# Kamino666/video_features

Measured on NVIDIA H100. Metric: frames/sec CLIP-ViT-B/32 @224px, higher is better.
Workload: dtype f16

## Files before the change

video_features_b200/csrc/attn_gemm.cu:

```cuda
#include <string.h>

#include <atomic>

#include "common.cuh"
#include "internal.h"
#include "wgmma.cuh"

namespace vf {

namespace {

constexpr int BM = 128, BK = 64, BN = 192, STAGES = 4;
constexpr int FRAMES_PER_TILE = 2, TOK = 50, TILE_ROWS = FRAMES_PER_TILE * TOK;
constexpr int THREADS = 384, CONSUMER_THREADS = 256, CONSUMER_WARPS = 8;
constexpr uint32_t A_BYTES = BM * BK * 2, B_BYTES = BN * BK * 2, STAGE_BYTES = A_BYTES + B_BYTES;
constexpr int PITCH = 200;
constexpr uint32_t STG_BYTES = BM * PITCH * 2;
constexpr uint32_t ZERO_BYTES = 128;
constexpr uint32_t BAR_BYTES = 2 * STAGES * 8;
constexpr uint32_t SMEM_BYTES = STAGES * STAGE_BYTES + STG_BYTES + ZERO_BYTES + BAR_BYTES + 1024;
static_assert(SMEM_BYTES <= 227 * 1024, "shared memory budget");

__device__ __forceinline__ void mma16816(float* c, const uint32_t* a, uint32_t b0, uint32_t b1) {
    asm volatile(
        "mma.sync.aligned.m16n8k16.row.col.f32.f16.f16.f32 {%0,%1,%2,%3}, {%4,%5,%6,%7}, {%8,%9}, {%0,%1,%2,%3};"
        : "+f"(c[0]), "+f"(c[1]), "+f"(c[2]), "+f"(c[3])
        : "r"(a[0]), "r"(a[1]), "r"(a[2]), "r"(a[3]), "r"(b0), "r"(b1));
}
__device__ __forceinline__ void ldsm_x4(uint32_t* r, const void* p) {
    asm volatile("ldmatrix.sync.aligned.m8n8.x4.shared.b16 {%0,%1,%2,%3}, [%4];"
                 : "=r"(r[0]), "=r"(r[1]), "=r"(r[2]), "=r"(r[3]) : "r"(smem_u32(p)));
}
__device__ __forceinline__ void ldsm_x4_trans(uint32_t* r, const void* p) {
    asm volatile("ldmatrix.sync.aligned.m8n8.x4.trans.shared.b16 {%0,%1,%2,%3}, [%4];"
                 : "=r"(r[0]), "=r"(r[1]), "=r"(r[2]), "=r"(r[3]) : "r"(smem_u32(p)));
}
__device__ __forceinline__ void attention_unit(__half* S, const __half* zero, int qrow0, int krow0, int nvalid, int lane) {
    const int g = lane >> 2, t = lane & 3;
    uint32_t aq[4][4];
#pragma unroll
    for (int ks = 0; ks < 4; ++ks) ldsm_x4(aq[ks], S + (qrow0 + (lane & 15)) * PITCH + ks * 16 + (lane >> 4) * 8);
    float s[8][4];
#pragma unroll
    for (int nt = 0; nt < 7; ++nt) {
        s[nt][0] = s[nt][1] = s[nt][2] = s[nt][3] = 0.f;
#pragma unroll
        for (int kp = 0; kp < 2; ++kp) {
            uint32_t bk[4];
            const int kr = nt * 8 + (lane & 7);
            ldsm_x4(bk, kr < TOK ? S + (krow0 + kr) * PITCH + 64 + kp * 32 + (lane >> 3) * 8 : zero);
            mma16816(s[nt], aq[2 * kp], bk[0], bk[1]);
            mma16816(s[nt], aq[2 * kp + 1], bk[2], bk[3]);
        }
    }
    const float sc = 0.125f * 1.4426950408889634f;
    float m_lo = -INFINITY, m_hi = -INFINITY;
#pragma unroll
    for (int nt = 0; nt < 7; ++nt) {
#pragma unroll
        for (int j = 0; j < 2; ++j) {
            const bool valid = nt * 8 + 2 * t + j < TOK;
            s[nt][j] = valid ? s[nt][j] * sc : -INFINITY;
            s[nt][2 + j] = valid ? s[nt][2 + j] * sc : -INFINITY;
            m_lo = fmaxf(m_lo, s[nt][j]);
            m_hi = fmaxf(m_hi, s[nt][2 + j]);
        }
    }
    m_lo = fmaxf(m_lo, __shfl_xor_sync(0xffffffffu, m_lo, 1));
    m_lo = fmaxf(m_lo, __shfl_xor_sync(0xffffffffu, m_lo, 2));
    m_hi = fmaxf(m_hi, __shfl_xor_sync(0xffffffffu, m_hi, 1));
    m_hi = fmaxf(m_hi, __shfl_xor_sync(0xffffffffu, m_hi, 2));
    float sum_lo = 0.f, sum_hi = 0.f;
#pragma unroll
    for (int nt = 0; nt < 7; ++nt) {
#pragma unroll
        for (int j = 0; j < 2; ++j) {
            s[nt][j] = exp2f(s[nt][j] - m_lo);
            s[nt][2 + j] = exp2f(s[nt][2 + j] - m_hi);
            sum_lo += s[nt][j];
            sum_hi += s[nt][2 + j];
        }
    }
    s[7][0] = s[7][1] = s[7][2] = s[7][3] = 0.f;
    sum_lo += __shfl_xor_sync(0xffffffffu, sum_lo, 1);
    sum_lo += __shfl_xor_sync(0xffffffffu, sum_lo, 2);
    sum_hi += __shfl_xor_sync(0xffffffffu, sum_hi, 1);
    sum_hi += __shfl_xor_sync(0xffffffffu, sum_hi, 2);
    const float inv_lo = 1.0f / sum_lo, inv_hi = 1.0f / sum_hi;
    uint32_t pa[4][4];
#pragma unroll
    for (int kk = 0; kk < 4; ++kk) {
        pa[kk][0] = pack_half2(s[2 * kk][0] * inv_lo, s[2 * kk][1] * inv_lo);
        pa[kk][1] = pack_half2(s[2 * kk][2] * inv_hi, s[2 * kk][3] * inv_hi);
        pa[kk][2] = pack_half2(s[2 * kk + 1][0] * inv_lo, s[2 * kk + 1][1] * inv_lo);
        pa[kk][3] = pack_half2(s[2 * kk + 1][2] * inv_hi, s[2 * kk + 1][3] * inv_hi);
    }
    __syncwarp();
#pragma unroll
    for (int np = 0; np < 4; ++np) {
        float o0[4] = {0.f, 0.f, 0.f, 0.f}, o1[4] = {0.f, 0.f, 0.f, 0.f};
#pragma unroll
        for (int kk = 0; kk < 4; ++kk) {
            uint32_t bv[4];
            const int vr = kk * 16 + (lane & 7) + ((lane >> 3) & 1) * 8;
            ldsm_x4_trans(bv, vr < TOK ? S + (krow0 + vr) * PITCH + 128 + np * 16 + (lane >> 4) * 8 : zero);
            mma16816(o0, pa[kk], bv[0], bv[1]);
            mma16816(o1, pa[kk], bv[2], bv[3]);
        }
        if (g < nvalid) {
            *reinterpret_cast<uint32_t*>(S + (qrow0 + g) * PITCH + np * 16 + 2 * t) = pack_half2(o0[0], o0[1]);
            *reinterpret_cast<uint32_t*>(S + (qrow0 + g) * PITCH + np * 16 + 8 + 2 * t) = pack_half2(o1[0], o1[1]);
        }
        if (g + 8 < nvalid) {
            *reinterpret_cast<uint32_t*>(S + (qrow0 + g + 8) * PITCH + np * 16 + 2 * t) = pack_half2(o0[2], o0[3]);
            *reinterpret_cast<uint32_t*>(S + (qrow0 + g + 8) * PITCH + np * 16 + 8 + 2 * t) = pack_half2(o1[2], o1[3]);
        }
    }
    __syncwarp();
}

__global__ void __launch_bounds__(THREADS, 1)
qkv_attention_kernel(const __grid_constant__ CUtensorMap tmA, const __grid_constant__ CUtensorMap tmB,
                     const float* __restrict__ bias, __half* __restrict__ att, const int n_frames, const int heads) {
    extern __shared__ uint8_t smem_raw[];
    uint8_t* smem = reinterpret_cast<uint8_t*>((reinterpret_cast<uintptr_t>(smem_raw) + 1023) & ~uintptr_t(1023));
    uint8_t* sA = smem;
    uint8_t* sB = smem + STAGES * A_BYTES;
    __half* S = reinterpret_cast<__half*>(smem + STAGES * STAGE_BYTES);
    __half* zero = reinterpret_cast<__half*>(smem + STAGES * STAGE_BYTES + STG_BYTES);
    uint64_t* full = reinterpret_cast<uint64_t*>(smem + STAGES * STAGE_BYTES + STG_BYTES + ZERO_BYTES);
    uint64_t* empty = full + STAGES;

    const int warp = threadIdx.x >> 5, lane = threadIdx.x & 31;
    const int num_m = (n_frames + FRAMES_PER_TILE - 1) / FRAMES_PER_TILE;
    const int num_tiles = num_m * heads;
    const int width = heads * 64;
    constexpr int num_k = 768 / BK;

    if (threadIdx.x == 0) {
        tma_prefetch_desc(&tmA);
        tma_prefetch_desc(&tmB);
        for (int i = 0; i < STAGES; ++i) {
            mbar_init(&full[i], 1);
            mbar_init(&empty[i], CONSUMER_WARPS);
        }
        fence_mbar_init();
    }
    if (threadIdx.x < ZERO_BYTES / 16) reinterpret_cast<uint4*>(zero)[threadIdx.x] = make_uint4(0, 0, 0, 0);
    __syncthreads();

    if (warp < 4) {
        if (warp == 0 && lane == 0) {
            int stage = 0;
            uint32_t phase = 0;
            for (int tile = blockIdx.x; tile < num_tiles; tile += gridDim.x) {
                const int m0 = (tile % num_m) * TILE_ROWS;
                const int n0 = (tile / num_m) * BN;
                for (int kk = 0; kk < num_k; ++kk) {
                    mbar_wait(&empty[stage], phase ^ 1);
                    mbar_expect_tx(&full[stage], STAGE_BYTES);
                    tma_load_2d(sA + stage * A_BYTES, &tmA, &full[stage], kk * BK, m0);
                    tma_load_2d(sB + stage * B_BYTES, &tmB, &full[stage], kk * BK, n0);
                    if (++stage == STAGES) { stage = 0; phase ^= 1; }
                }
            }
        }
        return;
    }

    const int wg = (warp >> 2) - 1, wq = warp & 3;
    const int e = warp - 4;
    const int f = e >> 2, tok0 = (e & 3) * 16;
    const int krow0 = TOK * f, qrow0 = krow0 + tok0;
    float acc[BN / 2];
    int stage = 0;
    uint32_t phase = 0;
    for (int tile = blockIdx.x; tile < num_tiles; tile += gridDim.x) {
        const int m_blk = tile % num_m, head = tile / num_m;
        int prev = -1;
        for (int kb = 0; kb < num_k; ++kb) {
            mbar_wait(&full[stage], phase);
            const uint64_t adesc = wgmma_desc_sw128(sA + stage * A_BYTES + wg * (64 * 128));
            const uint64_t bdesc = wgmma_desc_sw128(sB + stage * B_BYTES);
            wgmma_fence_regs<BN / 2>(acc);
            wgmma_fence();
#pragma unroll
            for (int k = 0; k < BK / 16; ++k) Wgmma<BN>::mma(acc, adesc + 2 * k, bdesc + 2 * k, (kb | k) != 0 ? 1u : 0u);
            wgmma_commit();
            wgmma_wait<1>();
            wgmma_fence_regs<BN / 2>(acc);
            if (prev >= 0) {
                __syncwarp();
                if (lane == 0) mbar_arrive(&empty[prev]);
            }
            prev = stage;
            if (++stage == STAGES) { stage = 0; phase ^= 1; }
        }
        wgmma_wait<0>();
        wgmma_fence_regs<BN / 2>(acc);
        __syncwarp();
        if (lane == 0) mbar_arrive(&empty[prev]);

        named_bar_sync(1, CONSUMER_THREADS);
        const float* hb = bias + head * BN;
#pragma unroll
        for (int j = 0; j < BN / 8; ++j) {
            const int c = 8 * j + 2 * (lane & 3);
            const float2 b = __ldg(reinterpret_cast<const float2*>(hb + c));
#pragma unroll
            for (int h = 0; h < 2; ++h) {
                const int r = wg * 64 + wq * 16 + (lane >> 2) + 8 * h;
                *reinterpret_cast<uint32_t*>(S + r * PITCH + c) = pack_half2(acc[4 * j + 2 * h] + b.x, acc[4 * j + 2 * h + 1] + b.y);
            }
        }
        named_bar_sync(1, CONSUMER_THREADS);
        attention_unit(S, zero, qrow0, krow0, tok0 + 16 <= TOK ? 16 : TOK - tok0, lane);
        const int frame = m_blk * FRAMES_PER_TILE + f;
        if (frame < n_frames) {
            __half* orow = att + (int64_t(frame) * TOK) * width + head * 64;
#pragma unroll
            for (int i = 0; i < 4; ++i) {
                const int r = i * 4 + (lane >> 3), seg = lane & 7;
                const int tok = tok0 + r;
                if (tok < TOK)
                    *reinterpret_cast<uint4*>(orow + int64_t(tok) * width + seg * 8) =
                        *reinterpret_cast<const uint4*>(S + (qrow0 + r) * PITCH + seg * 8);
            }
        }
    }
}

}

int qkv_attention(const __half* h, int lda, const __half* w_perm, const float* bias_perm, __half* att, int n_frames, int heads,
                  cudaStream_t stream) {
    if (n_frames <= 0) return VF_OK;
    if (heads * 64 != 768) return fail(VF_ERR_UNSUPPORTED, "qkv_attention: built for width 768 (heads * 64)");
    static std::atomic<bool> attr_set[64];
    int dev = 0;
    VF_CUDA(cudaGetDevice(&dev));
    if (dev < 0 || dev >= 64 || !attr_set[dev].load(std::memory_order_acquire)) {
        VF_CUDA(cudaFuncSetAttribute(qkv_attention_kernel, cudaFuncAttributeMaxDynamicSharedMemorySize, SMEM_BYTES));
        if (dev >= 0 && dev < 64) attr_set[dev].store(true, std::memory_order_release);
    }
    const int M = n_frames * TOK;
    CUtensorMap tmA, tmB;
    VF_TRY(make_tmap_2d(&tmA, h, 2, uint64_t(M), 768, uint64_t(lda) * 2, BM, BK));
    VF_TRY(make_tmap_2d(&tmB, w_perm, 2, uint64_t(heads) * BN, 768, 768 * 2, BN, BK));
    const int tiles = ((n_frames + FRAMES_PER_TILE - 1) / FRAMES_PER_TILE) * heads;
    const int sms = device_sm_count();
    const int grid = tiles < sms ? tiles : sms;
    qkv_attention_kernel<<<grid, THREADS, SMEM_BYTES, stream>>>(tmA, tmB, bias_perm, att, n_frames, heads);
    VF_CUDA(cudaGetLastError());
    return VF_OK;
}

}
```

Before: 46370.

## Warp-specialize fused QKV-attention kernel with MMA/attention overlap via staging ring

Splits the consumer role into one MMA warpgroup, which computes full 128-row QKV tiles with two accumulators, and two attention warpgroups. They hand off through a double-buffered shared-memory ring guarded by staged/freed mbarriers, so the GEMM for the next tile runs while attention works on the previous one. Tiles now pack contiguous frames (128 rows instead of 100), and each CTA is pinned to one head over a contiguous frame range, so the weight slice and bias (now cached in shared memory) stay resident. Register budgets are rebalanced with setmaxnreg and pipeline stages drop from 4 to 3 to fit the ring. The risks are fewer stages, a high register demand for the MMA warps, and frames that straddle tile boundaries, which adds extra waits.

```diff
diff --git a/video_features_b200/csrc/attn_gemm.cu b/video_features_b200/csrc/attn_gemm.cu
--- a/video_features_b200/csrc/attn_gemm.cu
+++ b/video_features_b200/csrc/attn_gemm.cu
@@ -10,16 +10,32 @@
 
 namespace {
 
-constexpr int BM = 128, BK = 64, BN = 192, STAGES = 4;
-constexpr int FRAMES_PER_TILE = 2, TOK = 50, TILE_ROWS = FRAMES_PER_TILE * TOK;
-constexpr int THREADS = 384, CONSUMER_THREADS = 256, CONSUMER_WARPS = 8;
+constexpr int BM = 128, BK = 64, BN = 192, STAGES = 3;
+constexpr int TOK = 50;
+constexpr int THREADS = 512, MMA_WARPS = 4, ATT_WARPS = 8;
+constexpr uint32_t PRODUCER_REGS = 40, MMA_REGS = 232, ATT_REGS = 120;
+static_assert(PRODUCER_REGS + MMA_REGS + 2 * ATT_REGS == 4 * 128, "register split");
 constexpr uint32_t A_BYTES = BM * BK * 2, B_BYTES = BN * BK * 2, STAGE_BYTES = A_BYTES + B_BYTES;
 constexpr int PITCH = 200;
-constexpr uint32_t STG_BYTES = BM * PITCH * 2;
+constexpr int RING = 2 * BM;
+constexpr uint32_t STG_BYTES = RING * PITCH * 2;
 constexpr uint32_t ZERO_BYTES = 128;
-constexpr uint32_t BAR_BYTES = 2 * STAGES * 8;
-constexpr uint32_t SMEM_BYTES = STAGES * STAGE_BYTES + STG_BYTES + ZERO_BYTES + BAR_BYTES + 1024;
+constexpr uint32_t BIAS_BYTES = BN * 4;
+constexpr uint32_t BAR_BYTES = (2 * STAGES + 4) * 8;
+constexpr uint32_t SMEM_BYTES = STAGES * STAGE_BYTES + STG_BYTES + ZERO_BYTES + BIAS_BYTES + BAR_BYTES + 1024;
 static_assert(SMEM_BYTES <= 227 * 1024, "shared memory budget");
+
+struct FrameRange {
+    int frame0, frames, tiles;
+};
+__device__ __forceinline__ FrameRange frame_range(int n_frames, int cph, int r) {
+    const int base = n_frames / cph, rem = n_frames % cph;
+    FrameRange g;
+    g.frame0 = r * base + (r < rem ? r : rem);
+    g.frames = base + (r < rem ? 1 : 0);
+    g.tiles = (g.frames * TOK + BM - 1) / BM;
+    return g;
+}
 
 __device__ __forceinline__ void mma16816(float* c, const uint32_t* a, uint32_t b0, uint32_t b1) {
     asm volatile(
@@ -35,11 +51,13 @@
     asm volatile("ldmatrix.sync.aligned.m8n8.x4.trans.shared.b16 {%0,%1,%2,%3}, [%4];"
                  : "=r"(r[0]), "=r"(r[1]), "=r"(r[2]), "=r"(r[3]) : "r"(smem_u32(p)));
 }
+__device__ __forceinline__ __half* ring_row(__half* S, int r) { return S + (r & (RING - 1)) * PITCH; }
 __device__ __forceinline__ void attention_unit(__half* S, const __half* zero, int qrow0, int krow0, int nvalid, int lane) {
     const int g = lane >> 2, t = lane & 3;
     uint32_t aq[4][4];
 #pragma unroll
-    for (int ks = 0; ks < 4; ++ks) ldsm_x4(aq[ks], S + (qrow0 + (lane & 15)) * PITCH + ks * 16 + (lane >> 4) * 8);
+    for (int ks = 0; ks < 4; ++ks)
+        ldsm_x4(aq[ks], (lane & 15) < nvalid ? ring_row(S, qrow0 + (lane & 15)) + ks * 16 + (lane >> 4) * 8 : zero);
     float s[8][4];
 #pragma unroll
     for (int nt = 0; nt < 7; ++nt) {
@@ -48,7 +66,7 @@
         for (int kp = 0; kp < 2; ++kp) {
             uint32_t bk[4];
             const int kr = nt * 8 + (lane & 7);
-            ldsm_x4(bk, kr < TOK ? S + (krow0 + kr) * PITCH + 64 + kp * 32 + (lane >> 3) * 8 : zero);
+            ldsm_x4(bk, kr < TOK ? ring_row(S, krow0 + kr) + 64 + kp * 32 + (lane >> 3) * 8 : zero);
             mma16816(s[nt], aq[2 * kp], bk[0], bk[1]);
             mma16816(s[nt], aq[2 * kp + 1], bk[2], bk[3]);
         }
@@ -103,17 +121,17 @@
         for (int kk = 0; kk < 4; ++kk) {
             uint32_t bv[4];
             const int vr = kk * 16 + (lane & 7) + ((lane >> 3) & 1) * 8;
-            ldsm_x4_trans(bv, vr < TOK ? S + (krow0 + vr) * PITCH + 128 + np * 16 + (lane >> 4) * 8 : zero);
+            ldsm_x4_trans(bv, vr < TOK ? ring_row(S, krow0 + vr) + 128 + np * 16 + (lane >> 4) * 8 : zero);
             mma16816(o0, pa[kk], bv[0], bv[1]);
             mma16816(o1, pa[kk], bv[2], bv[3]);
         }
         if (g < nvalid) {
-            *reinterpret_cast<uint32_t*>(S + (qrow0 + g) * PITCH + np * 16 + 2 * t) = pack_half2(o0[0], o0[1]);
-            *reinterpret_cast<uint32_t*>(S + (qrow0 + g) * PITCH + np * 16 + 8 + 2 * t) = pack_half2(o1[0], o1[1]);
+            *reinterpret_cast<uint32_t*>(ring_row(S, qrow0 + g) + np * 16 + 2 * t) = pack_half2(o0[0], o0[1]);
+            *reinterpret_cast<uint32_t*>(ring_row(S, qrow0 + g) + np * 16 + 8 + 2 * t) = pack_half2(o1[0], o1[1]);
         }
         if (g + 8 < nvalid) {
-            *reinterpret_cast<uint32_t*>(S + (qrow0 + g + 8) * PITCH + np * 16 + 2 * t) = pack_half2(o0[2], o0[3]);
-            *reinterpret_cast<uint32_t*>(S + (qrow0 + g + 8) * PITCH + np * 16 + 8 + 2 * t) = pack_half2(o1[2], o1[3]);
+            *reinterpret_cast<uint32_t*>(ring_row(S, qrow0 + g + 8) + np * 16 + 2 * t) = pack_half2(o0[2], o0[3]);
+            *reinterpret_cast<uint32_t*>(ring_row(S, qrow0 + g + 8) + np * 16 + 8 + 2 * t) = pack_half2(o1[2], o1[3]);
         }
     }
     __syncwarp();
@@ -121,20 +139,26 @@
 
 __global__ void __launch_bounds__(THREADS, 1)
 qkv_attention_kernel(const __grid_constant__ CUtensorMap tmA, const __grid_constant__ CUtensorMap tmB,
-                     const float* __restrict__ bias, __half* __restrict__ att, const int n_frames, const int heads) {
+                     const float* __restrict__ bias, __half* __restrict__ att, const int n_frames, const int heads,
+                     const int cph) {
+    const int head = blockIdx.x % heads;
+    const FrameRange rg = frame_range(n_frames, cph, blockIdx.x / heads);
+    if (rg.frames <= 0) return;
+
     extern __shared__ uint8_t smem_raw[];
     uint8_t* smem = reinterpret_cast<uint8_t*>((reinterpret_cast<uintptr_t>(smem_raw) + 1023) & ~uintptr_t(1023));
     uint8_t* sA = smem;
     uint8_t* sB = smem + STAGES * A_BYTES;
     __half* S = reinterpret_cast<__half*>(smem + STAGES * STAGE_BYTES);
     __half* zero = reinterpret_cast<__half*>(smem + STAGES * STAGE_BYTES + STG_BYTES);
-    uint64_t* full = reinterpret_cast<uint64_t*>(smem + STAGES * STAGE_BYTES + STG_BYTES + ZERO_BYTES);
+    float* sbias = reinterpret_cast<float*>(smem + STAGES * STAGE_BYTES + STG_BYTES + ZERO_BYTES);
+    uint64_t* full = reinterpret_cast<uint64_t*>(smem + STAGES * STAGE_BYTES + STG_BYTES + ZERO_BYTES + BIAS_BYTES);
     uint64_t* empty = full + STAGES;
+    uint64_t* staged = empty + STAGES;
+    uint64_t* freed = staged + 2;
 
     const int warp = threadIdx.x >> 5, lane = threadIdx.x & 31;
-    const int num_m = (n_frames + FRAMES_PER_TILE - 1) / FRAMES_PER_TILE;
-    const int num_tiles = num_m * heads;
-    const int width = heads * 64;
+    const int row0 = rg.frame0 * TOK;
     constexpr int num_k = 768 / BK;
 
     if (threadIdx.x == 0) {
@@ -142,25 +166,30 @@
         tma_prefetch_desc(&tmB);
         for (int i = 0; i < STAGES; ++i) {
             mbar_init(&full[i], 1);
-            mbar_init(&empty[i], CONSUMER_WARPS);
+            mbar_init(&empty[i], MMA_WARPS);
+        }
+        for (int i = 0; i < 2; ++i) {
+            mbar_init(&staged[i], MMA_WARPS);
+            mbar_init(&freed[i], ATT_WARPS);
         }
         fence_mbar_init();
     }
     if (threadIdx.x < ZERO_BYTES / 16) reinterpret_cast<uint4*>(zero)[threadIdx.x] = make_uint4(0, 0, 0, 0);
+    if (threadIdx.x < BN) sbias[threadIdx.x] = bias[head * BN + threadIdx.x];
     __syncthreads();
 
     if (warp < 4) {
+        setmaxnreg_dec<PRODUCER_REGS>();
         if (warp == 0 && lane == 0) {
             int stage = 0;
             uint32_t phase = 0;
-            for (int tile = blockIdx.x; tile < num_tiles; tile += gridDim.x) {
-                const int m0 = (tile % num_m) * TILE_ROWS;
-                const int n0 = (tile / num_m) * BN;
+            for (int t = 0; t < rg.tiles; ++t) {
+                const int m0 = row0 + t * BM;
                 for (int kk = 0; kk < num_k; ++kk) {
                     mbar_wait(&empty[stage], phase ^ 1);
                     mbar_expect_tx(&full[stage], STAGE_BYTES);
                     tma_load_2d(sA + stage * A_BYTES, &tmA, &full[stage], kk * BK, m0);
-                    tma_load_2d(sB + stage * B_BYTES, &tmB, &full[stage], kk * BK, n0);
+                    tma_load_2d(sB + stage * B_BYTES, &tmB, &full[stage], kk * BK, head * BN);
                     if (++stage == STAGES) { stage = 0; phase ^= 1; }
                 }
             }
@@ -168,27 +197,63 @@
         return;
     }
 
-    const int wg = (warp >> 2) - 1, wq = warp & 3;
-    const int e = warp - 4;
-    const int f = e >> 2, tok0 = (e & 3) * 16;
-    const int krow0 = TOK * f, qrow0 = krow0 + tok0;
-    float acc[BN / 2];
+    if (warp >= 8) {
+        setmaxnreg_dec<ATT_REGS>();
+        const int aw = warp - 8;
+        const int tok0 = (aw & 3) * 16, nvalid = tok0 + 16 <= TOK ? 16 : TOK - tok0;
+        const int width = heads * 64;
+        int waited = 0, released = 0;
+        auto hand_back = [&] {
+            if (waited == released) {
+                mbar_wait(&staged[released & 1], (released >> 1) & 1);
+                ++waited;
+            }
+            if (lane == 0) mbar_arrive(&freed[released & 1]);
+            ++released;
+        };
+        for (int j = aw >> 2; j < rg.frames; j += 2) {
+            const int r0 = j * TOK;
+            while ((released + 1) * BM <= r0) hand_back();
+            for (const int t_hi = (r0 + TOK - 1) / BM; waited <= t_hi; ++waited)
+                mbar_wait(&staged[waited & 1], (waited >> 1) & 1);
+            attention_unit(S, zero, r0 + tok0, r0, nvalid, lane);
+            __half* orow = att + int64_t(row0 + r0) * width + head * 64;
+#pragma unroll
+            for (int i = 0; i < 4; ++i) {
+                const int r = i * 4 + (lane >> 3), seg = lane & 7;
+                if (r < nvalid)
+                    *reinterpret_cast<uint4*>(orow + int64_t(tok0 + r) * width + seg * 8) =
+                        *reinterpret_cast<const uint4*>(ring_row(S, r0 + tok0 + r) + seg * 8);
+            }
+            __syncwarp();
+        }
+        while (released < rg.tiles) hand_back();
+        return;
+    }
+
+    setmaxnreg_inc<MMA_REGS>();
+    const int wq = warp & 3;
+    float acc[2][BN / 2];
     int stage = 0;
     uint32_t phase = 0;
-    for (int tile = blockIdx.x; tile < num_tiles; tile += gridDim.x) {
-        const int m_blk = tile % num_m, head = tile / num_m;
+    for (int t = 0; t < rg.tiles; ++t) {
         int prev = -1;
         for (int kb = 0; kb < num_k; ++kb) {
             mbar_wait(&full[stage], phase);
-            const uint64_t adesc = wgmma_desc_sw128(sA + stage * A_BYTES + wg * (64 * 128));
+            const uint64_t adesc = wgmma_desc_sw128(sA + stage * A_BYTES);
             const uint64_t bdesc = wgmma_desc_sw128(sB + stage * B_BYTES);
-            wgmma_fence_regs<BN / 2>(acc);
+            wgmma_fence_regs<BN / 2>(acc[0]);
+            wgmma_fence_regs<BN / 2>(acc[1]);
             wgmma_fence();
 #pragma unroll
-            for (int k = 0; k < BK / 16; ++k) Wgmma<BN>::mma(acc, adesc + 2 * k, bdesc + 2 * k, (kb | k) != 0 ? 1u : 0u);
+            for (int k = 0; k < BK / 16; ++k) {
+                Wgmma<BN>::mma(acc[0], adesc + 2 * k, bdesc + 2 * k, (kb | k) != 0 ? 1u : 0u);
+                Wgmma<BN>::mma(acc[1], adesc + (64 * 128 >> 4) + 2 * k, bdesc + 2 * k, (kb | k) != 0 ? 1u : 0u);
+            }
             wgmma_commit();
             wgmma_wait<1>();
-            wgmma_fence_regs<BN / 2>(acc);
+            wgmma_fence_regs<BN / 2>(acc[0]);
+            wgmma_fence_regs<BN / 2>(acc[1]);
             if (prev >= 0) {
                 __syncwarp();
                 if (lane == 0) mbar_arrive(&empty[prev]);
@@ -197,36 +262,30 @@
             if (++stage == STAGES) { stage = 0; phase ^= 1; }
         }
         wgmma_wait<0>();
-        wgmma_fence_regs<BN / 2>(acc);
+        wgmma_fence_regs<BN / 2>(acc[0]);
+        wgmma_fence_regs<BN / 2>(acc[1]);
         __syncwarp();
         if (lane == 0) mbar_arrive(&empty[prev]);
 
-        named_bar_sync(1, CONSUMER_THREADS);
-        const float* hb = bias + head * BN;
-#pragma unroll
-        for (int j = 0; j < BN / 8; ++j) {
-            const int c = 8 * j + 2 * (lane & 3);
-            const float2 b = __ldg(reinterpret_cast<const float2*>(hb + c));
-#pragma unroll
-            for (int h = 0; h < 2; ++h) {
-                const int r = wg * 64 + wq * 16 + (lane >> 2) + 8 * h;
-                *reinterpret_cast<uint32_t*>(S + r * PITCH + c) = pack_half2(acc[4 * j + 2 * h] + b.x, acc[4 * j + 2 * h + 1] + b.y);
-            }
-        }
-        named_bar_sync(1, CONSUMER_THREADS);
-        attention_unit(S, zero, qrow0, krow0, tok0 + 16 <= TOK ? 16 : TOK - tok0, lane);
-        const int frame = m_blk * FRAMES_PER_TILE + f;
-        if (frame < n_frames) {
-            __half* orow = att + (int64_t(frame) * TOK) * width + head * 64;
-#pragma unroll
-            for (int i = 0; i < 4; ++i) {
-                const int r = i * 4 + (lane >> 3), seg = lane & 7;
-                const int tok = tok0 + r;
-                if (tok < TOK)
-                    *reinterpret_cast<uint4*>(orow + int64_t(tok) * width + seg * 8) =
-                        *reinterpret_cast<const uint4*>(S + (qrow0 + r) * PITCH + seg * 8);
-            }
-        }
+        if (t >= 2) mbar_wait(&freed[t & 1], ((t >> 1) - 1) & 1);
+        __half* T = S + (t & 1) * BM * PITCH;
+#pragma unroll
+        for (int m = 0; m < 2; ++m) {
+            asm volatile("" ::: "memory");
+#pragma unroll
+            for (int j = 0; j < BN / 8; ++j) {
+                const int c = 8 * j + 2 * (lane & 3);
+                const float2 b = *reinterpret_cast<const float2*>(sbias + c);
+#pragma unroll
+                for (int h = 0; h < 2; ++h) {
+                    const int r = m * 64 + wq * 16 + (lane >> 2) + 8 * h;
+                    *reinterpret_cast<uint32_t*>(T + r * PITCH + c) =
+                        pack_half2(acc[m][4 * j + 2 * h] + b.x, acc[m][4 * j + 2 * h + 1] + b.y);
+                }
+            }
+        }
+        __syncwarp();
+        if (lane == 0) mbar_arrive(&staged[t & 1]);
     }
 }
 
@@ -247,10 +306,10 @@
     CUtensorMap tmA, tmB;
     VF_TRY(make_tmap_2d(&tmA, h, 2, uint64_t(M), 768, uint64_t(lda) * 2, BM, BK));
     VF_TRY(make_tmap_2d(&tmB, w_perm, 2, uint64_t(heads) * BN, 768, 768 * 2, BN, BK));
-    const int tiles = ((n_frames + FRAMES_PER_TILE - 1) / FRAMES_PER_TILE) * heads;
-    const int sms = device_sm_count();
-    const int grid = tiles < sms ? tiles : sms;
-    qkv_attention_kernel<<<grid, THREADS, SMEM_BYTES, stream>>>(tmA, tmB, bias_perm, att, n_frames, heads);
+    int cph = device_sm_count() / heads;
+    if (cph > n_frames) cph = n_frames;
+    if (cph < 1) cph = 1;
+    qkv_attention_kernel<<<cph * heads, THREADS, SMEM_BYTES, stream>>>(tmA, tmB, bias_perm, att, n_frames, heads, cph);
     VF_CUDA(cudaGetLastError());
     return VF_OK;
 }
```

New measurement: 48060 (median of 6 runs). +3.7%, better.
